# agakshat/spacefortress

Measured on NVIDIA B200. Metric: env-steps/sec with 84x84 obs, higher is better.
Workload: dtype f64

## Files before the change

spacefortress_b200/csrc/sf_kernels.cu:

```cuda
#include <cuda_runtime.h>
#include <stdio.h>
#include <stdlib.h>
#include <string.h>

#include <algorithm>
#include <mutex>
#include <string>
#include <vector>

#include "../../include/sf_b200.h"
#include "sf_geom.h"
#include "sf_render.cuh"
#include "sf_state.cuh"
#include "sf_step.cuh"
#include "sf_tables.h"

#define SF_BLOCK (32 * SF_RENDER_WARPS)

__host__ __device__ inline unsigned sf_hash3(unsigned seed, unsigned long long env, unsigned long long t) {
  unsigned long long z = (env * 0x9E3779B97F4A7C15ull) ^ (t * 0xC2B2AE3D27D4EB4Full) ^ ((unsigned long long)seed << 32 | 0x5Fu);
  z ^= z >> 30; z *= 0xBF58476D1CE4E5B9ull;
  z ^= z >> 27; z *= 0x94D049BB133111EBull;
  z ^= z >> 31;
  return (unsigned)(z >> 32);
}
__host__ __device__ inline int sf_hash_action(unsigned seed, unsigned long long env, unsigned long long t, int num_actions) {
  return (int)(((unsigned long long)sf_hash3(seed, env, t) * (unsigned)num_actions) >> 32);
}

__device__ __forceinline__ long long sf_warp_sum_ll(long long v) {
// ... 68 lines not shown
  unsigned long long* delta_stats;
  const unsigned char* draw_mask;
};
struct SfFeatArgs {
  float* out;
  int kind, cols;
};
enum SfRollMode { SF_ROLL_STEP, SF_ROLL_STEP_HOST_DELTA, SF_ROLL_DRAW };
template <int MODE>
__device__ __forceinline__ int sf_roll_ticks(const SfRollArgs& A) { return MODE == SF_ROLL_DRAW ? 1 : A.T; }

__device__ __forceinline__ int sf_step_keys(const SfDev& D, const SfRollArgs& A, int env, int t) {
  int a = A.actions ? A.actions[(size_t)t * D.n + env]
                    : sf_hash_action(A.action_seed, (unsigned long long)(D.first_global_env + env), (unsigned long long)(A.t0 + t), D.num_actions);
  return (A.flags & SF_FLAG_ACTIONS_ARE_KEYMASKS) ? (a & 15) : D.keymask_of_action[min(max(a, 0), D.num_actions - 1)];
}
__device__ __forceinline__ void sf_store_step_out(const SfDev& D, const SfRollArgs& A, int env, int t, const SfStepOut& o) {
  size_t oi = (size_t)t * D.n + env;
  if (A.reward) A.reward[oi] = o.reward;
  if (A.done) A.done[oi] = o.done;
  if (A.fortkill) A.fortkill[oi] = o.fort_kill;
  if (A.events) A.events[oi] = o.events;
}
__device__ __forceinline__ void sf_tick_env(const SfDev& D, const SfHot* H, const SfRollArgs& A, int env, int t, bool autoreset, SfEnv& e, SfStepOut& o) {
  const int km = sf_step_keys(D, A, env, t);
  sf_env_step(D, H, env, e, km, autoreset, (A.flags & SF_FLAG_RAW_REWARD) != 0, o);
  sf_store_step_out(D, A, env, t, o);
}

__device__ __noinline__ void sf_step_group(const SfDev& D, const SfRollArgs& A, int group, int t, SfEnvRec* recs) {
  const int lane = threadIdx.x & 31;
  const SfHot* H = &sf_block_smem().hot;
  const bool autoreset = !(A.flags & SF_FLAG_NO_AUTORESET);
  const int env = A.env0 + group * A.EB + lane;
  const bool mine = lane < A.EB && env < A.env0 + A.envn;
  SfEnv e;
  bool finished = false;
  unsigned shell_vis = 0;
  SF_ST_BEGIN(__ballot_sync(0xffffffffu, mine));
  SfStepSmem& SS = sf_block_smem().step;
  const bool first_tick = t == 0, last_tick = t == A.T - 1;
  if (mine) {
    if (first_tick) sf_load_env(D, env, e);
    else {
      e.pos = SS.pos[lane]; e.vel = SS.vel[lane];
      e.q0 = SS.q0[lane]; e.q1 = SS.q1[lane]; e.q2 = SS.q2[lane]; e.q3 = SS.q3[lane]; e.st3 = SS.st3[lane];
      e.d0 = SS.d0[lane]; e.d1 = SS.d1[lane]; e.d2 = SS.d2[lane];
    }
    SF_ST_USE(e.q0.x, e.q0.y);
    SF_ST(8);
    SfStepOut o;
    sf_tick_env(D, H, A, env, t, autoreset, e, o);
    finished = o.done && autoreset;
    shell_vis = o.shell_vis;
  }
  SF_ST_RESTART(0xffffffffu);
  if (__any_sync(0xffffffffu, finished)) {
    sf_accumulate_episode(D, env, e, finished, lane);
    if (finished) { sf_new_game(D, H, env, e); shell_vis = 0; }
  }
  if (mine) {
    if (last_tick) sf_store_env(D, env, e);
    else {
      SS.pos[lane] = e.pos; SS.vel[lane] = e.vel;
      SS.q0[lane] = e.q0; SS.q1[lane] = e.q1; SS.q2[lane] = e.q2; SS.q3[lane] = e.q3; SS.st3[lane] = e.st3;
      if ((t & 7) == 7) sf_flush_stats(D, env, e);
      SS.d0[lane] = e.d0; SS.d1[lane] = e.d1; SS.d2[lane] = e.d2;
    }
    sf_make_env_rec(e, env, shell_vis, recs[lane]);
  } else recs[lane].env = -1;
  __syncwarp();
  SF_ST(15);
}

__device__ __forceinline__ void sf_load_group(const SfDev& D, const SfRollArgs& A, int group, SfEnvRec* recs) {
  const int lane = threadIdx.x & 31;
  const int env = A.env0 + group * A.EB + lane;
  const bool mine = lane < A.EB && env < A.env0 + A.envn && (!A.draw_mask || A.draw_mask[env]);
  if (mine) {
    SfEnv e;
    sf_load_env(D, env, e);
    sf_make_env_rec(e, env, sf_visible_shells(D, env, (unsigned)e.q0.y), recs[lane]);
  } else recs[lane].env = -1;
  __syncwarp();
}

template <int MODE>
__device__ __forceinline__ void sf_stepper_role(const SfDev& D, const SfRollArgs& A) {
  const int lane = threadIdx.x & 31;
  SfBlockSmem& B = sf_block_smem();
  const bool native = (A.flags & SF_FLAG_NATIVE_OBS) != 0;
  int stage = 0, group = blockIdx.x;
#pragma unroll 1
  for (int k = 0; group < A.ngroups; k = (k + 1) % SF_NEXT_GROUPS) {
    if (lane == 0) B.next_group[k] = A.sched ? (int)gridDim.x + atomicAdd(&A.sched->next_group, 1) : group + (int)gridDim.x;
    sf_stepper_ticks(D, B, lane, native, sf_roll_ticks<MODE>(A), stage, [&](int t, SfStagePrep& Tm, int h) {
      if constexpr (MODE == SF_ROLL_DRAW) sf_load_group(D, A, group, Tm.env);
      else sf_step_group(D, A, group, t, &Tm.env[32 * h]);
    });
    group = B.next_group[k];
  }
  sf_stepper_drain(stage);
  if (lane == 0 && A.sched) {
    __threadfence();
    if (atomicAdd(&A.sched->done, 1) == (int)gridDim.x - 1) { A.sched->next_group = 0; A.sched->done = 0; __threadfence(); }
  }
}
template <int MODE>
__device__ __noinline__ void sf_rollout_stepper(const SfDev& D, const SfRollArgs& A) { sf_stepper_role<MODE>(D, A); }

template <int MODE>
__device__ __forceinline__ void sf_rollout_drawer(const SfDev& D, const SfRollArgs& A) {
  const int lane = threadIdx.x & 31;
  SfBlockSmem& B = sf_block_smem();
  SfWarpSmem& W = sf_my_smem();
  SfFrameOut out;
  out.native = (A.flags & SF_FLAG_NATIVE_OBS) ? 1 : 0;
  out.obs_bytes = out.native ? (size_t)SF_NAT_H * SF_NAT_W : (size_t)84 * 84;
  out.obs = A.obs;
  out.tick_bytes = MODE == SF_ROLL_DRAW ? 0 : (size_t)D.n * out.obs_bytes;
  SfStageState st;
// ... 352 lines not shown
  D.st1[i] = make_int4(r.stats[4], r.stats[5], r.stats[6], r.stats[7]);
  D.st2[i] = make_int4(r.stats[8], r.stats[9], r.stats[10], r.stats[11]);
  e.st3.x = r.stats[12];
  for (int s = 0; s < SF_MAX_MISSILES; s++) if ((r.missile_mask >> s) & 1) {
    D.mpos[(size_t)s * D.n_pad + i] = make_double2(r.missile_x[s], r.missile_y[s]);
    D.mang[(size_t)s * D.n_pad + i] = (short)(int)r.missile_angle[s];
  }
  for (int s = 0; s < SF_DEV_SHELLS; s++) if ((r.shell_mask >> s) & 1) {
    D.spos[(size_t)s * D.n_pad + i] = make_double2(r.shell_x[s], r.shell_y[s]);
    D.svel[(size_t)s * D.n_pad + i] = make_double2(r.shell_vx[s], r.shell_vy[s]);
    D.sang[(size_t)s * D.n_pad + i] = r.shell_angle[s];
  }
  sf_forget_render_caches(D, i);
  sf_store_env(D, i, e);
}

#define SF_BLOB_CHUNKS (SF_ENV_BLOB_BYTES / 16)
#define SF_BLOB_PITCH (SF_BLOB_CHUNKS + 1)
#define SF_BLOB_BLOCKS_PER_SM 8
enum { SF_BO_POS = 16, SF_BO_VEL = 32, SF_BO_Q = 48, SF_BO_ST = 112, SF_BO_MPOS = 176, SF_BO_SPOS = 496, SF_BO_SVEL = 560,
       SF_BO_SANG = 624, SF_BO_MANG = 656, SF_BO_RNG = 696, SF_BO_END = 820 };
static_assert(SF_BO_MANG + 2 * SF_MAX_MISSILES == SF_BO_RNG && SF_BO_RNG + 4 * SF_RNG_WORDS == SF_BO_END, "blob layout");
static_assert(SF_BO_END <= SF_ENV_BLOB_BYTES && SF_ENV_BLOB_BYTES % 16 == 0, "blob size");

__device__ __forceinline__ void sf_cp_async(void* smem, const void* gmem, int bytes) {
  const unsigned s = (unsigned)__cvta_generic_to_shared(smem);
  if (bytes == 16) asm volatile("cp.async.cg.shared.global [%0], [%1], 16;\n" ::"r"(s), "l"(gmem) : "memory");
  else if (bytes == 8) asm volatile("cp.async.ca.shared.global [%0], [%1], 8;\n" ::"r"(s), "l"(gmem) : "memory");
  else asm volatile("cp.async.ca.shared.global [%0], [%1], 4;\n" ::"r"(s), "l"(gmem) : "memory");
}
__device__ __forceinline__ void sf_cp_async_wait() { asm volatile("cp.async.wait_all;\n" ::: "memory"); }

__global__ void __launch_bounds__(32) sf_save_envs_kernel(SfDev D, int gametype, const int* __restrict__ idx, int count, int4* __restrict__ blob) {
  __shared__ int4 tile[32 * SF_BLOB_PITCH];
  const int lane = threadIdx.x;
  const size_t np = (size_t)D.n_pad;
  int4* row = tile + lane * SF_BLOB_PITCH;
  char* rb = reinterpret_cast<char*>(row);
  const int4 z = make_int4(0, 0, 0, 0);
  for (int base = blockIdx.x * 32; base < count; base += gridDim.x * 32) {
    const int k = base + lane;
    const int i = k < count ? (idx ? idx[k] : k) : -1;
    if (i >= 0 && i < D.n) {
      const int4 q0 = D.q0[i];
      const unsigned pm = (unsigned)q0.y;
      row[0] = make_int4((int)SF_ENV_BLOB_MAGIC, SF_ENV_BLOB_VERSION, gametype, 0);
      sf_cp_async(rb + SF_BO_POS, &D.pos[i], 16);
      sf_cp_async(rb + SF_BO_VEL, &D.vel[i], 16);
      row[SF_BO_Q / 16] = q0;
      sf_cp_async(rb + SF_BO_Q + 16, &D.q1[i], 16);
      sf_cp_async(rb + SF_BO_Q + 32, &D.q2[i], 16);
      sf_cp_async(rb + SF_BO_Q + 48, &D.q3[i], 16);
      sf_cp_async(rb + SF_BO_ST, &D.st0[i], 16);
      sf_cp_async(rb + SF_BO_ST + 16, &D.st1[i], 16);
// ... 235 lines not shown
  d.autoturn = (gt == 1 || gt == 3);
  bool test = gt >= 2;
  d.shaped = !test;
  d.destroy_fortress = test ? 100 : 1;
  d.death_penalty = test ? 100 : 1;
  d.missile_penalty = test ? 2.0f : (float)0.05;
  d.num_actions = na;
  for (int i = 0; i < 16; i++) d.keymask_of_action[i] = i < na ? km[i] : 0;
  d.first_global_env = 0;

  h->h_tab = new SfTables();
  char err[256] = {0};
  if (sf_build_tables(h->h_tab, err, sizeof(err))) { std::string m = err; delete h->h_tab; delete h; return fail(SF_ERR_INVALID, "table build failed: " + m); }

  auto bail = [&](const char* what, cudaError_t ce) { std::string m = std::string(what) + ": " + cudaGetErrorString(ce); sf_destroy(h); return fail(SF_ERR_CUDA, m); };
  cudaError_t ce;
  h->slab_bytes = layout(d, nullptr);
  if ((ce = cudaMalloc(&h->slab, h->slab_bytes)) != cudaSuccess) return bail("cudaMalloc state slab", ce);
  layout(d, (char*)h->slab);
  if ((ce = cudaMalloc(&h->d_sched, sizeof(SfSched))) != cudaSuccess) return bail("cudaMalloc scheduler state", ce);
  if ((ce = cudaMemset(h->d_sched, 0, sizeof(SfSched))) != cudaSuccess) return bail("cudaMemset scheduler state", ce);
  if ((ce = cudaMemset(h->slab, 0, h->slab_bytes)) != cudaSuccess) return bail("cudaMemset state slab", ce);
  if ((ce = cudaMemcpy((void*)d.tab, h->h_tab, sizeof(SfTables), cudaMemcpyHostToDevice)) != cudaSuccess) return bail("upload tables", ce);
  if ((ce = cudaFuncSetAttribute(sf_rollout_kernel<SF_ROLL_STEP>, cudaFuncAttributeMaxDynamicSharedMemorySize, (int)SF_RENDER_SMEM_BYTES(SF_RENDER_WARPS))) != cudaSuccess) return bail("shared memory opt-in (rollout)", ce);
  if ((ce = cudaFuncSetAttribute(sf_rollout_kernel<SF_ROLL_STEP_HOST_DELTA>, cudaFuncAttributeMaxDynamicSharedMemorySize, (int)SF_RENDER_SMEM_BYTES(SF_RENDER_WARPS))) != cudaSuccess) return bail("shared memory opt-in (rollout, host delta)", ce);
  if ((ce = cudaFuncSetAttribute(sf_rollout_kernel<SF_ROLL_DRAW>, cudaFuncAttributeMaxDynamicSharedMemorySize, (int)SF_RENDER_SMEM_BYTES(SF_RENDER_WARPS))) != cudaSuccess) return bail("shared memory opt-in (rollout, draw)", ce);
  if ((ce = cudaFuncSetAttribute(sf_pack_static_kernel, cudaFuncAttributeMaxDynamicSharedMemorySize, (int)SF_RENDER_SMEM_BYTES(SF_RENDER_WARPS))) != cudaSuccess) return bail("shared memory opt-in (pack)", ce);
  if ((ce = cudaFuncSetAttribute(sf_save_envs_kernel, cudaFuncAttributePreferredSharedMemoryCarveout, (int)cudaSharedmemCarveoutMaxShared)) != cudaSuccess) return bail("shared memory carveout (save envs)", ce);
  if ((ce = cudaFuncSetAttribute(sf_load_envs_kernel, cudaFuncAttributePreferredSharedMemoryCarveout, (int)cudaSharedmemCarveoutMaxShared)) != cudaSuccess) return bail("shared memory carveout (load envs)", ce);
  sf_pack_static_kernel<<<1, SF_BLOCK, SF_RENDER_SMEM_BYTES(SF_RENDER_WARPS)>>>(d, const_cast<unsigned char*>(d.static_image));
  if ((ce = cudaGetLastError()) != cudaSuccess) return bail("static image kernel launch", ce);
  sf_seed_kernel<<<(d.n + 127) / 128, 128>>>(d, nullptr);
  if ((ce = cudaGetLastError()) != cudaSuccess) return bail("seed kernel launch", ce);
  if ((ce = cudaDeviceSynchronize()) != cudaSuccess) return bail("seed kernel", ce);
  *out = h;
  return SF_OK;
}

extern "C" int sf_destroy(sf_handle* h) {
  if (!h) return SF_OK;
  cudaSetDevice(h->device);
  if (h->slab) cudaFree(h->slab);
  if (h->d_actions) cudaFree(h->d_actions);
  if (h->d_obs) cudaFree(h->d_obs);
  if (h->d_reward) cudaFree(h->d_reward);
  if (h->d_done) cudaFree(h->d_done);
  if (h->d_kill) cudaFree(h->d_kill);
// ... 62 lines not shown
      if (render) {
        const size_t o = (size_t)t * n;
        s.actions = a.actions ? a.actions + o : nullptr; s.t0 = a.t0 + t;
        s.reward = a.reward ? a.reward + o : nullptr; s.done = a.done ? a.done + o : nullptr;
        s.fortkill = a.fortkill ? a.fortkill + o : nullptr; s.events = a.events ? a.events + o : nullptr;
      }
      if (f.out) sf_step_repeat_kernel<true><<<blocks, SF_STEP_ONLY_BLOCK, 0, st>>>(d, s, f, h->action_repeat);
      else sf_step_repeat_kernel<false><<<blocks, SF_STEP_ONLY_BLOCK, 0, st>>>(d, s, f, h->action_repeat);
      CUDA_TRY(cudaGetLastError());
      if (render) {
        SfRollArgs r = {};
        r.T = 1; r.obs = a.obs + (size_t)t * n * per; r.flags = a.flags; r.env0 = a.env0; r.envn = a.envn;
        if (int rc = launch_rollout(h, r, st, true)) return rc;
      }
    }
    return SF_OK;
  }
  if (render) {
    int blocks;
    group_shape(h, a.envn, &a.EB, &a.ngroups, &blocks);
    a.sched = (!draw && a.env0 == 0 && a.envn == d.n && !a.host_obs) ? h->d_sched : nullptr;
    if (draw) sf_rollout_kernel<SF_ROLL_DRAW><<<blocks, SF_BLOCK, SF_RENDER_SMEM_BYTES(SF_RENDER_WARPS), st>>>(d, a);
    else if (a.host_obs) sf_rollout_kernel<SF_ROLL_STEP_HOST_DELTA><<<blocks, SF_BLOCK, SF_RENDER_SMEM_BYTES(SF_RENDER_WARPS), st>>>(d, a);
    else sf_rollout_kernel<SF_ROLL_STEP><<<blocks, SF_BLOCK, SF_RENDER_SMEM_BYTES(SF_RENDER_WARPS), st>>>(d, a);
  } else {
    const int blocks = (a.envn + SF_STEP_ONLY_BLOCK - 1) / SF_STEP_ONLY_BLOCK;
    if (f.out) sf_step_only_kernel<true><<<blocks, SF_STEP_ONLY_BLOCK, 0, st>>>(d, a, f);
    else sf_step_only_kernel<false><<<blocks, SF_STEP_ONLY_BLOCK, 0, st>>>(d, a, f);
  }
  CUDA_TRY(cudaGetLastError());
  return SF_OK;
}

#include <cuda_bf16.h>
#define SF_PI_THREADS 192
template <bool F32>
__global__ void __launch_bounds__(SF_PI_THREADS) sf_policy_input_kernel(const unsigned char* __restrict__ frames, long long fstride, int n, const int* __restrict__ valid,
                                                                       uint4* __restrict__ out) {
  __shared__ unsigned tile[2][4 * 4 * 21];
  __shared__ unsigned lut[256];
  const int env = blockIdx.x, tid = threadIdx.x;
  for (int v = tid; v < 256; v += SF_PI_THREADS) {
    if (F32) lut[v] = __float_as_uint(__fmul_rn((float)v, __fdiv_rn(1.0f, 255.0f)));
    else { const __nv_bfloat16 h = __float2bfloat16_rn(__fdiv_rn((float)v, 255.0f)); lut[v] = *reinterpret_cast<const unsigned short*>(&h); }
  }
  const int nvalid = min(max(valid[env], 0), 4);
  const unsigned char* base = frames + (long long)env * (84 * 84);
// ... 415 lines not shown
```

spacefortress_b200/csrc/sf_render.cuh:

```cuda
#pragma once
#include "sf_geom.h"
#include "sf_probe.cuh"
#include "sf_state.cuh"
#include "sf_tables.h"

#define SF_BATCH_QUADS 32
#define SF_MAX_GROUPS 256
#define SF_PATCH_STRIDE 32
#define SF_PATCH_BYTES (36 * 32)
#define SF_WIN_MAX_W 31
#define SF_WIN_MAX_H 34
#define SF_YBIAS 4096
#define SF_TAG_SHIP 0
#define SF_TAG_PROJECTILE 1
#define SF_SPAN_NONE 0xFFFFFFFFu
#define SF_QF_IRREGULAR 2

#define SF_RENDER_WARPS 24
#define SF_FORT_LIST_SMEM 48
#define SF_GROUP_ENVS 32
#define SF_STAGE_TICKS 2
#define SF_STAGE_SLOTS (SF_GROUP_ENVS * SF_STAGE_TICKS)
#define SF_ROUND_STROKES (8 * (SF_RENDER_WARPS - 1))
#define SF_CELLS_SHIP 144
// ... 100 lines not shown
  asm volatile("bar.arrive %0, %1;" :: "r"(3 + sg), "r"(32 * SF_RENDER_WARPS) : "memory");
}
__device__ __forceinline__ void sf_stage_full_wait(int sg) {
  SF_BT_BEGIN();
  asm volatile("bar.sync %0, %1;" :: "r"(3 + sg), "r"(32 * SF_RENDER_WARPS) : "memory");
  SF_BT(0);
}
__device__ __forceinline__ void sf_stage_empty_arrive(int sg) {
  asm volatile("bar.arrive %0, %1;" :: "r"(3 + SF_PREP_SLOTS + sg), "r"(32 * SF_RENDER_WARPS) : "memory");
}
__device__ __forceinline__ void sf_stage_empty_wait(int sg) {
  SF_BT_BEGIN();
  asm volatile("bar.sync %0, %1;" :: "r"(3 + SF_PREP_SLOTS + sg), "r"(32 * SF_RENDER_WARPS) : "memory");
  SF_BT(2);
}
__device__ __forceinline__ void sf_render_sync() {
  SF_BT_BEGIN();
  asm volatile("bar.sync 2, %0;" :: "r"(32 * (SF_RENDER_WARPS - 1)) : "memory");
  SF_BT(1);
}
__device__ __forceinline__ SfWarpSmem& sf_warp_smem(int warp) { return reinterpret_cast<SfWarpSmem*>(sf_smem_raw + sizeof(SfBlockSmem))[warp]; }
__device__ __forceinline__ SfWarpSmem& sf_my_smem() { return sf_warp_smem(threadIdx.x >> 5); }
#define SF_RENDER_SMEM_BYTES(warps) (sizeof(SfBlockSmem) + sizeof(SfWarpSmem) * (warps))

__device__ __forceinline__ int sf_warp_min(int v) {
#pragma unroll
  for (int o = 16; o; o >>= 1) v = min(v, __shfl_xor_sync(0xffffffffu, v, o));
  return v;
}
__device__ __forceinline__ int sf_warp_max(int v) {
#pragma unroll
  for (int o = 16; o; o >>= 1) v = max(v, __shfl_xor_sync(0xffffffffu, v, o));
  return v;
}
__device__ __forceinline__ int sf_div_small(int a, int b, float inv_b) {
  return __float2int_rz(((float)a + 0.5f) * inv_b);
}
__device__ __forceinline__ int sf_div15(int d) { return (d * 2185) >> 15; }

__device__ __forceinline__ void sf_block_smem_fill(const SfTables* T) {
  SfBlockSmem& B = sf_block_smem();
  for (int k = threadIdx.x; k < 168; k += blockDim.x) {
    const SfTap t = k < 84 ? T->xtap[k] : T->ytap[k - 84];
    int4 v = make_int4(t.si | (t.cnt << 8), __float_as_int(t.a[0]), __float_as_int(t.a[1]), __float_as_int(t.a[2]));
    if (k < 84) B.xtap[k] = v; else B.ytap[k - 84] = v;
  }
// ... 698 lines not shown
      for (int u = 0; u < 8; u++) {
        const int k = lane + 32 * u, w = k & 7;
        if (((rows >> (k >> 3)) & 1u) && w >= wfull0 && w < wfull1) *reinterpret_cast<unsigned*>(dst + (k >> 3) * 84 + 4 * w) = v[u];
      }
      if ((rows >> lane) & 1u) {
        const int wl = wfull0 - 1, wr = wfull1;
        if (wl >= 0) {
          const unsigned x = __ldcg(&src[lane * 8 + wl]);
          unsigned char* p = dst + lane * 84 + 4 * wl;
#pragma unroll
          for (int b = 0; b < 4; b++) { const int c = ja + 4 * wl + b; if (c >= j0 && c <= j1) p[b] = (unsigned char)(x >> (8 * b)); }
        }
        if (wr != wl && ja + 4 * wr <= j1) {
          const unsigned x = __ldcg(&src[lane * 8 + wr]);
          unsigned char* p = dst + lane * 84 + 4 * wr;
#pragma unroll
          for (int b = 0; b < 4; b++) { const int c = ja + 4 * wr + b; if (c >= j0 && c <= j1) p[b] = (unsigned char)(x >> (8 * b)); }
        }
      }
    }
  }
}

__device__ __forceinline__ void sf_gather_strokes(const SfDev& D, SfStagePrep& Tm, int lane, int h) {
  const int slot = 32 * h + lane;
  const SfEnvRec& rec = Tm.env[slot];
  if (slot >= Tm.r0 && slot < Tm.r1 && rec.env >= 0) {
    const int env = rec.env, np = D.n_pad;
    const unsigned core = rec.core;
    SfStrokeRec* S = &Tm.stroke[rec.s0];
    if (core & SF_CORE_SHIP_ALIVE) { S->x = rec.px; S->y = rec.py; S->desc = 0 | ((int)(core & SF_CORE_ANGLE_MASK) << 2) | (slot << 12); S++; }
    for (unsigned m = rec.pmask & SF_PMASK_MISSILES; m;) {
      const int k0 = __ffs(m) - 1; m &= m - 1;
      const int k1 = m ? __ffs(m) - 1 : k0; m &= m - 1;
      const int k2 = m ? __ffs(m) - 1 : k0; m &= m - 1;
      const double2 p0 = D.mpos[(size_t)k0 * np + env], p1 = D.mpos[(size_t)k1 * np + env], p2 = D.mpos[(size_t)k2 * np + env];
      const int a0 = D.mang[(size_t)k0 * np + env], a1 = D.mang[(size_t)k1 * np + env], a2 = D.mang[(size_t)k2 * np + env];
      S->x = p0.x; S->y = p0.y; S->desc = 1 | (a0 << 2) | (slot << 12); S++;
      if (k1 != k0) { S->x = p1.x; S->y = p1.y; S->desc = 1 | (a1 << 2) | (slot << 12); S++; }
      if (k2 != k0) { S->x = p2.x; S->y = p2.y; S->desc = 1 | (a2 << 2) | (slot << 12); S++; }
    }
    for (unsigned m = (unsigned)rec.shell_vis; m; m &= m - 1) {
      const int k = __ffs(m) - 1;
      const double2 p = D.spos[(size_t)k * np + env];
      int angle = __double2int_rz(D.sang[(size_t)k * np + env]);
      if (angle >= 360) angle -= 360;
      S->x = p.x; S->y = p.y; S->desc = 2 | (angle << 2) | (slot << 12); S++;
    }
  }
  __syncwarp();
}

__device__ __forceinline__ void sf_phase_strokes(const SfDev& D, SfBlockSmem& B, SfWarpSmem& W, int lane, int wi, int nw, int nst, int sg) {
  const SfTables* T = D.tab;
  const SfStagePrep& Tm = sf_prep(sg);
  const int chunk = Tm.chunk;
  const int be = Tm.build_env;
  if (be >= 0) sf_phase_exp_items(D, be, lane, nw - 1 - wi, nw, sg);
  const int s = wi * chunk;
  if (s < nst) {
    const int slot = lane >> 2;
    const bool valid = slot < chunk && s + slot < nst;
    const int idx = s + slot;
    int kind = -1, angle = 0;
    double x = 0, y = 0;
    if (valid) {
      const SfStrokeRec& S = Tm.stroke[idx];
      x = S.x; y = S.y; kind = S.desc & 3; angle = (S.desc >> 2) & 1023;
// ... 99 lines not shown
    for (int k = 0; k < SF_PREP_SLOTS * SF_STAGE_TICKS; k++) {
      const int j = k / SF_STAGE_TICKS, hh = k - j * SF_STAGE_TICKS;
      if (j == cur && hh >= h) continue;
      const SfEnvRec& o = ring[j].env[32 * hh + lane];
      if (o.env != r.env || (o.core & SF_CORE_SHIP_ALIVE)) continue;
      if (o.life == r.life) building = 0;
      if (o.life != r.life || sf_expo_key(o) != key) refresh = false;
    }
    if (!native) {
      const bool same = mx == r.life && (my & 0x0FFFFFFFu) == key;
      if (same) { if (!building) building |= (int)(my >> 28) << 4; }
      else atomicExch(reinterpret_cast<unsigned long long*>(&D.expo_meta[r.env]), (unsigned long long)r.life | ((unsigned long long)key << 32));
    }
    r.building = building | (refresh ? 2 : 0);
  }
  __syncwarp();
}

struct SfStageState {
  int stage;
  int prev_used;
};

template <class Prep>
__device__ __forceinline__ void sf_prepare_first_round(const SfDev& D, SfBlockSmem& B, int sg, int lane, int t, int nt, SfFrameOut out, Prep prep) {
  SfStagePrep& Tm = B.prep[sg];
  const bool native = out.native != 0;
  SF_BT_BEGIN();
  prep(t, Tm, 0);
  SF_BT(3);
  sf_publish_recs(D, B.prep, sg, lane, 0, native);
  SF_BT(4);
  SfScanState S;
  sf_scan_begin(S);
  sf_scan_half(Tm, lane, 0, 0, S);
  sf_scan_finish(Tm, lane, 0, S);
  SF_BT(5);
  sf_gather_strokes(D, Tm, lane, 0);
  SF_BT(6);
  int nticks = 1;
  if (nt > 1 && !Tm.more) {
    prep(t + 1, Tm, 1);
    SF_BT(3);
    sf_publish_recs(D, B.prep, sg, lane, 1, native);
    SF_BT(4);
    sf_scan_half(Tm, lane, 1, 0, S);
    sf_scan_finish(Tm, lane, 0, S);
    SF_BT(5);
    sf_gather_strokes(D, Tm, lane, 1);
    SF_BT(6);
    nticks = 2;
  }
  if (lane == 0) Tm.nticks = nticks;
  __syncwarp();
  SF_BT(7);
}

__device__ __forceinline__ int sf_draw_stage(const SfDev& D, SfBlockSmem& B, SfWarpSmem& W, int lane, const SfFrameOut& out, int sg) {
  const int warp = threadIdx.x >> 5;
  const int wi = warp - 1, nw = SF_RENDER_WARPS - 1;
  const SfStagePrep& Tm = B.prep[sg];
  SfStagePool& P = B.pool;
  const int r0 = Tm.r0, r1 = Tm.r1, nst = Tm.nstrokes;
  const bool base_issuer = !out.native && wi == nw - 1;
  if (base_issuer) {
#pragma unroll 1
    for (int e = r0 + lane; e < r1; e += 32) sf_env_base_issue(B, e, out, sg);
  }
  sf_phase_strokes(D, B, W, lane, wi, nw, nst, sg);
  if (!out.native) {
    if (base_issuer) {
      asm volatile("cp.async.bulk.wait_group 0;" ::: "memory");
// ... 26 lines not shown
      sf_phase_window(D, B, W, lane, t, netask, out, sg);
    }
  } else {
#pragma unroll 1
    for (int t = wi; t < (r1 - r0) * 12; t += nw) sf_phase_native_tile(D, B, W, lane, r0 + t / 12, t % 12, out, sg);
  }
  return used;
}


__device__ __forceinline__ int sf_stepper_claim(int stage) {
  const int sg = stage % SF_PREP_SLOTS;
  SF_TL(4);
  if (stage >= SF_PREP_SLOTS) sf_stage_empty_wait(sg);
  SF_TL(5);
  return sg;
}
__device__ __forceinline__ void sf_stepper_drain(int stage) {
#pragma unroll 1
  for (int s = max(stage - SF_PREP_SLOTS, 0); s < stage; s++)
    asm volatile("bar.sync %0, %1;" :: "r"(3 + SF_PREP_SLOTS + s % SF_PREP_SLOTS), "r"(32 * SF_RENDER_WARPS) : "memory");
}

template <class Prep>
__device__ __forceinline__ void sf_stepper_ticks(const SfDev& D, SfBlockSmem& B, int lane, bool native, int T, int& stage, Prep prep) {
  SfFrameOut out;
  out.obs = nullptr; out.obs_bytes = 0; out.tick_bytes = 0; out.native = native ? 1 : 0;
  int sg = sf_stepper_claim(stage);
  sf_prepare_first_round(D, B, sg, lane, 0, T, out, prep);
  SF_TL(3);
  int t = 0;
#pragma unroll 1
  for (;;) {
    sf_stage_full_arrive(sg);
    stage++;
    const SfStagePrep& Tm = B.prep[sg];
    const bool more = Tm.more != 0;
    const int nticks = Tm.nticks;
    if (!more && t + nticks >= T) break;
    const int nx = sf_stepper_claim(stage);
    SfStagePrep& Nx = B.prep[nx];
    if (more) {
#pragma unroll
      for (int h = 0; h < SF_STAGE_TICKS; h++) Nx.env[32 * h + lane] = Tm.env[32 * h + lane];
      if (lane == 0) Nx.nticks = nticks;
      __syncwarp();
      sf_round_scan(Nx, lane, Tm.r1, SF_GROUP_ENVS * nticks);
      sf_gather_strokes(D, Nx, lane, nticks - 1);
    } else {
      sf_prepare_first_round(D, B, nx, lane, t + nticks, T - (t + nticks), out, prep);
      t += nticks;
    }
    sg = nx;
  }
  SF_TL(7);
}

__device__ __forceinline__ void sf_drawer_ticks(const SfDev& D, SfBlockSmem& B, SfWarpSmem& W, int lane, SfFrameOut out, int T, SfStageState& st) {
  unsigned char* const obs0 = out.obs;
  int t = 0;
#pragma unroll 1
  for (;;) {
    const int sg = st.stage;
    SF_TL(4);
    sf_stage_full_wait(sg);
    SF_TL(5);
    const SfStagePrep& Tm = B.prep[sg];
    const bool more = Tm.more != 0;
    const int nticks = Tm.nticks;
    const bool last = !more && t + nticks >= T;
    {
      const int nz = (st.prev_used + 1) >> 1;
      for (int k = threadIdx.x - 32; k < nz; k += 32 * (SF_RENDER_WARPS - 1)) reinterpret_cast<unsigned*>(B.pool.cells)[k] = 0u;
// ... 12 lines not shown
```

spacefortress_b200/csrc/sf_state.cuh:

```cuda
#pragma once
#include <cuda_runtime.h>
#include <stdint.h>

#include "sf_tables.h"

#define SF_DEV_SHELLS 4
#define SF_RNG_WORDS 31

#define SF_CORE_ANGLE_MASK 0x1FFu
#define SF_CORE_FANG_SHIFT 9
#define SF_CORE_FLAST_SHIFT 15
#define SF_CORE_SHIP_ALIVE (1u << 21)
#define SF_CORE_FORT_ALIVE (1u << 22)
#define SF_CORE_FIRE (1u << 23)
#define SF_CORE_THRUST (1u << 24)
#define SF_CORE_LEFT (1u << 25)
#define SF_CORE_RIGHT (1u << 26)
#define SF_PMASK_MISSILES 0xFFFFFu
#define SF_PMASK_SHELL_SHIFT 20

struct SfDev {
  int n;
  int n_pad;
  double2* pos;
// ... 5 lines not shown
  int4* st0;
  int4* st1;
  int4* st2;
  int4* st3;
  double2* mpos;
  short* mang;
  double2* spos;
  double2* svel;
  double* sang;
  unsigned* rng;
  unsigned char* expc;
  unsigned* expstamp;
  unsigned char* expo;
  uint2* expo_meta;
  unsigned long long* epi;
  const SfTables* tab;
  const unsigned char* static_image;
  int autoturn, shaped, destroy_fortress, death_penalty;
  float missile_penalty;
  int num_actions;
  int keymask_of_action[16];
  long long first_global_env;
};
```

spacefortress_b200/csrc/sf_step.cuh:

```cuda
#pragma once
#include "sf_geom.h"
#include "sf_state.cuh"
#include "../../include/sf_b200.h"
#include "sf_probe.cuh"

#define SF_TICK_MS 34
#define SF_GAME_TIME 180000
#define SF_GAME_TICKS 5295

struct SfStepOut {
  int reward;
  unsigned events;
  bool done, fort_kill;
  unsigned shell_vis;
};

struct SfEnv {
  double2 pos, vel;
  int4 q0, q1, q2, q3, st3;
  unsigned d0, d1, d2;
};
#define SF_ST_INC(word, comp) ((word) += 1u << (8 * (comp)))

__device__ __forceinline__ void sf_load_env(const SfDev& D, int i, SfEnv& e) {
// ... 147 lines not shown
  e.st3.y = sp.w; e.st3.z += calls;
  e.pos = make_double2((double)sp.x, (double)sp.y);
  e.vel = make_double2(H->ship_start_vx, H->ship_start_vy);
  e.q0.x = (e.q0.x & ~SF_CORE_ANGLE_MASK) | (unsigned)sp.z | SF_CORE_SHIP_ALIVE;
}

__device__ inline void sf_new_game(const SfDev& D, const SfHot* H, int i, SfEnv& e) {
  e.q0 = make_int4(0, 0, 0, 0);
  sf_spawn_ship(D, H, i, e);
  e.q0.x |= SF_CORE_FORT_ALIVE | (18u << SF_CORE_FANG_SHIFT);
  e.q1 = make_int4(0, 250, 0, e.q1.w);
  e.q2 = make_int4(0, 0, 0, 0);
  e.q3 = make_int4(0, 0, 0, 0);
  D.st0[i] = make_int4(0, 0, 0, 0); D.st1[i] = make_int4(0, 0, 0, 0); D.st2[i] = make_int4(0, 0, 0, 0);
  e.d0 = 0u; e.d1 = 0u; e.d2 = 0u;
  e.st3.x = 0;
}

__device__ __forceinline__ int sf_first_free(unsigned mask, int n) {
  unsigned freebits = ~mask & ((1u << n) - 1u);
  return freebits ? __ffs(freebits) - 1 : -1;
}

__device__ inline void sf_env_step(const SfDev& D, const SfHot* T, int i, SfEnv& e, int keymask, bool autoreset, bool raw_reward, SfStepOut& out) {
  const int np = D.n_pad;
  SF_ST_BEGIN(__activemask());
  float rew = 0.f;
  unsigned ev = 0;
  unsigned core = (unsigned)e.q0.x;
  if (D.autoturn) keymask &= (SF_KEY_FIRE | SF_KEY_THRUST);

  {
    bool pressed = keymask & SF_KEY_FIRE, flag = core & SF_CORE_FIRE;
    if (pressed && !flag) {
      if (core & SF_CORE_SHIP_ALIVE) {
        int slot = sf_first_free((unsigned)e.q0.y & SF_PMASK_MISSILES, SF_MAX_MISSILES);
        if (slot >= 0) {
          e.q0.y |= 1 << slot;
          D.mpos[(size_t)slot * np + i] = e.pos;
          D.mang[(size_t)slot * np + i] = (short)(core & SF_CORE_ANGLE_MASK);
          ev |= SF_EV_MISSILE_FIRED;
          sf_reward(e, rew, -D.missile_penalty);
        }
      }
      core |= SF_CORE_FIRE; e.q2.x = 0; SF_ST_INC(e.d1, 3); ev |= SF_EV_PRESS_FIRE;
    } else if (!pressed && flag) { core &= ~SF_CORE_FIRE; e.q2.x = 0; }
    pressed = keymask & SF_KEY_THRUST; flag = core & SF_CORE_THRUST;
    if (pressed && !flag) { core |= SF_CORE_THRUST; e.q2.y = 0; SF_ST_INC(e.d2, 0); ev |= SF_EV_PRESS_THRUST; }
    else if (!pressed && flag) { core &= ~SF_CORE_THRUST; e.q2.y = 0; }
    if (!D.autoturn) {
      pressed = keymask & SF_KEY_LEFT; flag = core & SF_CORE_LEFT;
      if (pressed && !flag) { core |= SF_CORE_LEFT; e.q2.z = 0; SF_ST_INC(e.d2, 1); ev |= SF_EV_PRESS_LEFT; }
      else if (!pressed && flag) { core &= ~SF_CORE_LEFT; e.q2.z = 0; }
      pressed = keymask & SF_KEY_RIGHT; flag = core & SF_CORE_RIGHT;
      if (pressed && !flag) { core |= SF_CORE_RIGHT; e.q2.w = 0; SF_ST_INC(e.d2, 2); ev |= SF_EV_PRESS_RIGHT; }
      else if (!pressed && flag) { core &= ~SF_CORE_RIGHT; e.q2.w = 0; }
    }
  }
  e.q0.x = (int)core;

  if (!(core & SF_CORE_SHIP_ALIVE) && e.q0.z >= 1000) {
    sf_spawn_ship(D, T, i, e);
    e.q0.w = 0;
// ... 31 lines not shown
  }

  SF_ST(10);
  {
    if (!(core & SF_CORE_FORT_ALIVE) && e.q1.x > 1000) {
      e.q0.w = 0; core |= SF_CORE_FORT_ALIVE; ev |= SF_EV_FORTRESS_RESPAWN;
    }
    if (core & SF_CORE_SHIP_ALIVE) {
      const double fdy = SF_DSUB(e.pos.y, SF_FORT_Y), fdx = SF_DSUB(e.pos.x, SF_FORT_X);
      int sect = sf_ceil_angle<10>(T, fdy, fdx, false) / 10;
      if (sect >= 36) sect -= 36;
      unsigned last = (core >> SF_CORE_FLAST_SHIFT) & 63u;
      core = (core & ~(63u << SF_CORE_FANG_SHIFT)) | ((unsigned)sect << SF_CORE_FANG_SHIFT);
      if ((unsigned)sect != last) {
        core = (core & ~(63u << SF_CORE_FLAST_SHIFT)) | ((unsigned)sect << SF_CORE_FLAST_SHIFT);
        e.q0.w = 0;
      }
      if (e.q0.w >= 1000 && (core & SF_CORE_FORT_ALIVE)) {
        int slot = sf_first_free(((unsigned)e.q0.y >> SF_PMASK_SHELL_SHIFT) & 0xFu, SF_DEV_SHELLS);
        if (slot >= 0) {
          double a = sf_rad2deg(sf_atan2(T, fdy, fdx));
          if (a < 0) a = SF_DADD(a, 360.0);
          e.q0.y |= 1 << (SF_PMASK_SHELL_SHIFT + slot);
          D.spos[(size_t)slot * np + i] = make_double2(SF_FORT_X, SF_FORT_Y);
          D.svel[(size_t)slot * np + i] = sf_shell_velocity(a);
          D.sang[(size_t)slot * np + i] = a;
          ev |= SF_EV_FORTRESS_FIRED;
        }
        e.q0.w = 0;
      }
    }
    e.q0.x = (int)core;
  }

  SF_ST(11);
  const double thr_ship = T->touch2[0], thr_fort = T->touch2[1], thr_hide = T->touch2[2];
  unsigned vis = 0;
  for (unsigned m = ((unsigned)e.q0.y >> SF_PMASK_SHELL_SHIFT) & 0xFu; m; m &= m - 1) {
    int s = __ffs(m) - 1;
    double2 p = D.spos[(size_t)s * np + i], v = D.svel[(size_t)s * np + i];
    p.x = SF_DADD(p.x, v.x); p.y = SF_DADD(p.y, v.y);
    D.spos[(size_t)s * np + i] = p;
    if ((e.q0.x & SF_CORE_SHIP_ALIVE) && sf_dist2(p.x, p.y, e.pos.x, e.pos.y) <= thr_ship) {
      e.q0.y &= ~(1 << (SF_PMASK_SHELL_SHIFT + s));
      sf_kill_ship(e); sf_reward(e, rew, -(float)D.death_penalty); SF_ST_INC(e.d0, 2);
      ev |= SF_EV_SHELL_HIT_SHIP | SF_EV_COL_SHELL_SHIP;
    } else if (sf_outside(p.x, p.y)) {
      e.q0.y &= ~(1 << (SF_PMASK_SHELL_SHIFT + s));
    } else if (sf_dist2(p.x, p.y, SF_FORT_X, SF_FORT_Y) > thr_hide) vis |= 1u << s;
  }
  out.shell_vis = vis;

  SF_ST(12);
  for (unsigned m = (unsigned)e.q0.y & SF_PMASK_MISSILES; m; m &= m - 1) {
    int s = __ffs(m) - 1;
    double2 p = D.mpos[(size_t)s * np + i];
    int ang = D.mang[(size_t)s * np + i];
    p.x = SF_DADD(p.x, SF_DMUL(20.0, T->cs[ang][0]));
    p.y = SF_DADD(p.y, SF_DMUL(20.0, T->cs[ang][1]));
    D.mpos[(size_t)s * np + i] = p;
    if (sf_dist2(p.x, p.y, SF_FORT_X, SF_FORT_Y) <= thr_fort) {
      e.q0.y &= ~(1 << s);
      ev |= SF_EV_COL_MISSILE_FORTRESS;
      if (e.q0.x & SF_CORE_FORT_ALIVE) {
        ev |= SF_EV_HIT_FORTRESS;
        if (e.q1.y >= 250) {
          e.q1.z += 1; ev |= SF_EV_VLNER_INCREASED; SF_ST_INC(e.d2, 3);
          if (e.q1.z > e.st3.x) e.st3.x = e.q1.z;
        } else {
          if (e.q1.z >= 11) {
            e.q0.x &= ~SF_CORE_FORT_ALIVE; e.q1.x = 0;
            sf_reward(e, rew, (float)D.destroy_fortress);
            ev |= SF_EV_FORTRESS_DESTROYED; SF_ST_INC(e.d1, 1);
          } else { ev |= SF_EV_VLNER_RESET; SF_ST_INC(e.d1, 0); }
          e.q1.z = 0;
        }
        e.q1.y = 0;
      } else ev |= SF_EV_HIT_DEAD_FORTRESS;
    } else if (sf_outside(p.x, p.y)) {
      e.q0.y &= ~(1 << s);
      sf_reward(e, rew, -0.0f);
      SF_ST_INC(e.d1, 2); ev |= SF_EV_MISSED_SHOT;
    }
// ... 28 lines not shown
```

Baseline: 160.3 million.

## Keep projectile state in shared memory across rollout ticks

```diff
diff --git a/spacefortress_b200/csrc/sf_kernels.cu b/spacefortress_b200/csrc/sf_kernels.cu
--- a/spacefortress_b200/csrc/sf_kernels.cu
+++ b/spacefortress_b200/csrc/sf_kernels.cu
@@ -6,6 +6,7 @@
 #include <algorithm>
 #include <mutex>
 #include <string>
+#include <type_traits>
 #include <vector>
 
 #include "../../include/sf_b200.h"
@@ -120,12 +121,61 @@
   if (A.fortkill) A.fortkill[oi] = o.fort_kill;
   if (A.events) A.events[oi] = o.events;
 }
+template <class Proj = SfProjGlobal>
 __device__ __forceinline__ void sf_tick_env(const SfDev& D, const SfHot* H, const SfRollArgs& A, int env, int t, bool autoreset, SfEnv& e, SfStepOut& o) {
   const int km = sf_step_keys(D, A, env, t);
-  sf_env_step(D, H, env, e, km, autoreset, (A.flags & SF_FLAG_RAW_REWARD) != 0, o);
+  sf_env_step<Proj>(D, H, env, e, km, autoreset, (A.flags & SF_FLAG_RAW_REWARD) != 0, o);
   sf_store_step_out(D, A, env, t, o);
 }
 
+__device__ __forceinline__ void sf_cp_async(void* smem, const void* gmem, int bytes) {
+  const unsigned s = (unsigned)__cvta_generic_to_shared(smem);
+  if (bytes == 16) asm volatile("cp.async.cg.shared.global [%0], [%1], 16;\n" ::"r"(s), "l"(gmem) : "memory");
+  else if (bytes == 8) asm volatile("cp.async.ca.shared.global [%0], [%1], 8;\n" ::"r"(s), "l"(gmem) : "memory");
+  else asm volatile("cp.async.ca.shared.global [%0], [%1], 4;\n" ::"r"(s), "l"(gmem) : "memory");
+}
+__device__ __forceinline__ void sf_cp_async_wait() { asm volatile("cp.async.wait_all;\n" ::: "memory"); }
+
+__device__ __noinline__ void sf_proj_load(const SfDev& D, int env, unsigned pmask) {
+  SfProjSmem& P = sf_proj_smem();
+  const int lane = threadIdx.x & 31;
+  const size_t np = D.n_pad;
+  for (unsigned m = pmask & SF_PMASK_MISSILES; m; m &= m - 1) {
+    const int s = __ffs(m) - 1;
+    sf_cp_async(&P.mpos[s][lane], &D.mpos[s * np + env], 16);
+    sf_cp_async(&P.mang[s][lane], &D.mang[(s * np + env) & ~(size_t)1], 4);
+  }
+  for (unsigned m = (pmask >> SF_PMASK_SHELL_SHIFT) & 0xFu; m; m &= m - 1) {
+    const int s = __ffs(m) - 1;
+    sf_cp_async(&P.spos[s][lane], &D.spos[s * np + env], 16);
+    sf_cp_async(&P.svel[s][lane], &D.svel[s * np + env], 16);
+    sf_cp_async(&P.sang[s][lane], &D.sang[s * np + env], 8);
+  }
+  sf_cp_async_wait();
+  const int sh = (env & 1) ? 0 : 16;
+  for (unsigned m = pmask & SF_PMASK_MISSILES; m; m &= m - 1) {
+    const int s = __ffs(m) - 1;
+    P.mang[s][lane] = (int)((unsigned)P.mang[s][lane] << sh) >> 16;
+  }
+}
+__device__ __noinline__ void sf_proj_store(const SfDev& D, int env, unsigned pmask) {
+  const SfProjSmem& P = sf_proj_smem();
+  const int lane = threadIdx.x & 31;
+  const size_t np = D.n_pad;
+  for (unsigned m = pmask & SF_PMASK_MISSILES; m; m &= m - 1) {
+    const int s = __ffs(m) - 1;
+    D.mpos[s * np + env] = P.mpos[s][lane];
+    D.mang[s * np + env] = (short)P.mang[s][lane];
+  }
+  for (unsigned m = (pmask >> SF_PMASK_SHELL_SHIFT) & 0xFu; m; m &= m - 1) {
+    const int s = __ffs(m) - 1;
+    D.spos[s * np + env] = P.spos[s][lane];
+    D.svel[s * np + env] = P.svel[s][lane];
+    D.sang[s * np + env] = P.sang[s][lane];
+  }
+}
+
+template <class Proj>
 __device__ __noinline__ void sf_step_group(const SfDev& D, const SfRollArgs& A, int group, int t, SfEnvRec* recs) {
   const int lane = threadIdx.x & 31;
   const SfHot* H = &sf_block_smem().hot;
@@ -139,8 +189,10 @@
   SfStepSmem& SS = sf_block_smem().step;
   const bool first_tick = t == 0, last_tick = t == A.T - 1;
   if (mine) {
-    if (first_tick) sf_load_env(D, env, e);
-    else {
+    if (first_tick) {
+      sf_load_env(D, env, e);
+      if constexpr (std::is_same_v<Proj, SfProjShared>) sf_proj_load(D, env, (unsigned)e.q0.y);
+    } else {
       e.pos = SS.pos[lane]; e.vel = SS.vel[lane];
       e.q0 = SS.q0[lane]; e.q1 = SS.q1[lane]; e.q2 = SS.q2[lane]; e.q3 = SS.q3[lane]; e.st3 = SS.st3[lane];
       e.d0 = SS.d0[lane]; e.d1 = SS.d1[lane]; e.d2 = SS.d2[lane];
@@ -148,7 +200,7 @@
     SF_ST_USE(e.q0.x, e.q0.y);
     SF_ST(8);
     SfStepOut o;
-    sf_tick_env(D, H, A, env, t, autoreset, e, o);
+    sf_tick_env<Proj>(D, H, A, env, t, autoreset, e, o);
     finished = o.done && autoreset;
     shell_vis = o.shell_vis;
   }
@@ -158,8 +210,10 @@
     if (finished) { sf_new_game(D, H, env, e); shell_vis = 0; }
   }
   if (mine) {
-    if (last_tick) sf_store_env(D, env, e);
-    else {
+    if (last_tick) {
+      sf_store_env(D, env, e);
+      if constexpr (std::is_same_v<Proj, SfProjShared>) sf_proj_store(D, env, (unsigned)e.q0.y);
+    } else {
       SS.pos[lane] = e.pos; SS.vel[lane] = e.vel;
       SS.q0[lane] = e.q0; SS.q1[lane] = e.q1; SS.q2[lane] = e.q2; SS.q3[lane] = e.q3; SS.st3[lane] = e.st3;
       if ((t & 7) == 7) sf_flush_stats(D, env, e);
@@ -192,9 +246,10 @@
 #pragma unroll 1
   for (int k = 0; group < A.ngroups; k = (k + 1) % SF_NEXT_GROUPS) {
     if (lane == 0) B.next_group[k] = A.sched ? (int)gridDim.x + atomicAdd(&A.sched->next_group, 1) : group + (int)gridDim.x;
-    sf_stepper_ticks(D, B, lane, native, sf_roll_ticks<MODE>(A), stage, [&](int t, SfStagePrep& Tm, int h) {
+    using Proj = std::conditional_t<MODE == SF_ROLL_STEP, SfProjShared, SfProjGlobal>;
+    sf_stepper_ticks<Proj>(D, B, lane, native, sf_roll_ticks<MODE>(A), stage, [&](int t, SfStagePrep& Tm, int h) {
       if constexpr (MODE == SF_ROLL_DRAW) sf_load_group(D, A, group, Tm.env);
-      else sf_step_group(D, A, group, t, &Tm.env[32 * h]);
+      else sf_step_group<Proj>(D, A, group, t, &Tm.env[32 * h]);
     });
     group = B.next_group[k];
   }
@@ -593,14 +648,6 @@
        SF_BO_SANG = 624, SF_BO_MANG = 656, SF_BO_RNG = 696, SF_BO_END = 820 };
 static_assert(SF_BO_MANG + 2 * SF_MAX_MISSILES == SF_BO_RNG && SF_BO_RNG + 4 * SF_RNG_WORDS == SF_BO_END, "blob layout");
 static_assert(SF_BO_END <= SF_ENV_BLOB_BYTES && SF_ENV_BLOB_BYTES % 16 == 0, "blob size");
-
-__device__ __forceinline__ void sf_cp_async(void* smem, const void* gmem, int bytes) {
-  const unsigned s = (unsigned)__cvta_generic_to_shared(smem);
-  if (bytes == 16) asm volatile("cp.async.cg.shared.global [%0], [%1], 16;\n" ::"r"(s), "l"(gmem) : "memory");
-  else if (bytes == 8) asm volatile("cp.async.ca.shared.global [%0], [%1], 8;\n" ::"r"(s), "l"(gmem) : "memory");
-  else asm volatile("cp.async.ca.shared.global [%0], [%1], 4;\n" ::"r"(s), "l"(gmem) : "memory");
-}
-__device__ __forceinline__ void sf_cp_async_wait() { asm volatile("cp.async.wait_all;\n" ::: "memory"); }
 
 __global__ void __launch_bounds__(32) sf_save_envs_kernel(SfDev D, int gametype, const int* __restrict__ idx, int count, int4* __restrict__ blob) {
   __shared__ int4 tile[32 * SF_BLOB_PITCH];
@@ -882,7 +929,7 @@
   if ((ce = cudaMemset(h->d_sched, 0, sizeof(SfSched))) != cudaSuccess) return bail("cudaMemset scheduler state", ce);
   if ((ce = cudaMemset(h->slab, 0, h->slab_bytes)) != cudaSuccess) return bail("cudaMemset state slab", ce);
   if ((ce = cudaMemcpy((void*)d.tab, h->h_tab, sizeof(SfTables), cudaMemcpyHostToDevice)) != cudaSuccess) return bail("upload tables", ce);
-  if ((ce = cudaFuncSetAttribute(sf_rollout_kernel<SF_ROLL_STEP>, cudaFuncAttributeMaxDynamicSharedMemorySize, (int)SF_RENDER_SMEM_BYTES(SF_RENDER_WARPS))) != cudaSuccess) return bail("shared memory opt-in (rollout)", ce);
+  if ((ce = cudaFuncSetAttribute(sf_rollout_kernel<SF_ROLL_STEP>, cudaFuncAttributeMaxDynamicSharedMemorySize, (int)SF_ROLL_STEP_SMEM_BYTES)) != cudaSuccess) return bail("shared memory opt-in (rollout)", ce);
   if ((ce = cudaFuncSetAttribute(sf_rollout_kernel<SF_ROLL_STEP_HOST_DELTA>, cudaFuncAttributeMaxDynamicSharedMemorySize, (int)SF_RENDER_SMEM_BYTES(SF_RENDER_WARPS))) != cudaSuccess) return bail("shared memory opt-in (rollout, host delta)", ce);
   if ((ce = cudaFuncSetAttribute(sf_rollout_kernel<SF_ROLL_DRAW>, cudaFuncAttributeMaxDynamicSharedMemorySize, (int)SF_RENDER_SMEM_BYTES(SF_RENDER_WARPS))) != cudaSuccess) return bail("shared memory opt-in (rollout, draw)", ce);
   if ((ce = cudaFuncSetAttribute(sf_pack_static_kernel, cudaFuncAttributeMaxDynamicSharedMemorySize, (int)SF_RENDER_SMEM_BYTES(SF_RENDER_WARPS))) != cudaSuccess) return bail("shared memory opt-in (pack)", ce);
@@ -991,7 +1038,7 @@
     a.sched = (!draw && a.env0 == 0 && a.envn == d.n && !a.host_obs) ? h->d_sched : nullptr;
     if (draw) sf_rollout_kernel<SF_ROLL_DRAW><<<blocks, SF_BLOCK, SF_RENDER_SMEM_BYTES(SF_RENDER_WARPS), st>>>(d, a);
     else if (a.host_obs) sf_rollout_kernel<SF_ROLL_STEP_HOST_DELTA><<<blocks, SF_BLOCK, SF_RENDER_SMEM_BYTES(SF_RENDER_WARPS), st>>>(d, a);
-    else sf_rollout_kernel<SF_ROLL_STEP><<<blocks, SF_BLOCK, SF_RENDER_SMEM_BYTES(SF_RENDER_WARPS), st>>>(d, a);
+    else sf_rollout_kernel<SF_ROLL_STEP><<<blocks, SF_BLOCK, SF_ROLL_STEP_SMEM_BYTES, st>>>(d, a);
   } else {
     const int blocks = (a.envn + SF_STEP_ONLY_BLOCK - 1) / SF_STEP_ONLY_BLOCK;
     if (f.out) sf_step_only_kernel<true><<<blocks, SF_STEP_ONLY_BLOCK, 0, st>>>(d, a, f);
diff --git a/spacefortress_b200/csrc/sf_render.cuh b/spacefortress_b200/csrc/sf_render.cuh
--- a/spacefortress_b200/csrc/sf_render.cuh
+++ b/spacefortress_b200/csrc/sf_render.cuh
@@ -146,6 +146,23 @@
 __device__ __forceinline__ SfWarpSmem& sf_warp_smem(int warp) { return reinterpret_cast<SfWarpSmem*>(sf_smem_raw + sizeof(SfBlockSmem))[warp]; }
 __device__ __forceinline__ SfWarpSmem& sf_my_smem() { return sf_warp_smem(threadIdx.x >> 5); }
 #define SF_RENDER_SMEM_BYTES(warps) (sizeof(SfBlockSmem) + sizeof(SfWarpSmem) * (warps))
+
+struct __align__(16) SfProjSmem {
+  double2 mpos[SF_MAX_MISSILES][SF_GROUP_ENVS];
+  int mang[SF_MAX_MISSILES][SF_GROUP_ENVS];
+  double2 spos[SF_DEV_SHELLS][SF_GROUP_ENVS], svel[SF_DEV_SHELLS][SF_GROUP_ENVS];
+  double sang[SF_DEV_SHELLS][SF_GROUP_ENVS];
+};
+#define SF_ROLL_STEP_SMEM_BYTES (SF_RENDER_SMEM_BYTES(SF_RENDER_WARPS) + sizeof(SfProjSmem))
+__device__ __forceinline__ SfProjSmem& sf_proj_smem() { return *reinterpret_cast<SfProjSmem*>(sf_smem_raw + SF_RENDER_SMEM_BYTES(SF_RENDER_WARPS)); }
+struct SfProjShared {
+  static __device__ __forceinline__ double2& mpos(const SfDev&, int, int s, int) { return sf_proj_smem().mpos[s][threadIdx.x & 31]; }
+  static __device__ __forceinline__ int mang(const SfDev&, int, int s, int) { return sf_proj_smem().mang[s][threadIdx.x & 31]; }
+  static __device__ __forceinline__ void set_mang(const SfDev&, int, int s, int, int a) { sf_proj_smem().mang[s][threadIdx.x & 31] = a; }
+  static __device__ __forceinline__ double2& spos(const SfDev&, int, int s, int) { return sf_proj_smem().spos[s][threadIdx.x & 31]; }
+  static __device__ __forceinline__ double2& svel(const SfDev&, int, int s, int) { return sf_proj_smem().svel[s][threadIdx.x & 31]; }
+  static __device__ __forceinline__ double& sang(const SfDev&, int, int s, int) { return sf_proj_smem().sang[s][threadIdx.x & 31]; }
+};
 
 __device__ __forceinline__ int sf_warp_min(int v) {
 #pragma unroll
@@ -890,6 +907,7 @@
   }
 }
 
+template <class Proj>
 __device__ __forceinline__ void sf_gather_strokes(const SfDev& D, SfStagePrep& Tm, int lane, int h) {
   const int slot = 32 * h + lane;
   const SfEnvRec& rec = Tm.env[slot];
@@ -902,16 +920,16 @@
       const int k0 = __ffs(m) - 1; m &= m - 1;
       const int k1 = m ? __ffs(m) - 1 : k0; m &= m - 1;
       const int k2 = m ? __ffs(m) - 1 : k0; m &= m - 1;
-      const double2 p0 = D.mpos[(size_t)k0 * np + env], p1 = D.mpos[(size_t)k1 * np + env], p2 = D.mpos[(size_t)k2 * np + env];
-      const int a0 = D.mang[(size_t)k0 * np + env], a1 = D.mang[(size_t)k1 * np + env], a2 = D.mang[(size_t)k2 * np + env];
+      const double2 p0 = Proj::mpos(D, np, k0, env), p1 = Proj::mpos(D, np, k1, env), p2 = Proj::mpos(D, np, k2, env);
+      const int a0 = Proj::mang(D, np, k0, env), a1 = Proj::mang(D, np, k1, env), a2 = Proj::mang(D, np, k2, env);
       S->x = p0.x; S->y = p0.y; S->desc = 1 | (a0 << 2) | (slot << 12); S++;
       if (k1 != k0) { S->x = p1.x; S->y = p1.y; S->desc = 1 | (a1 << 2) | (slot << 12); S++; }
       if (k2 != k0) { S->x = p2.x; S->y = p2.y; S->desc = 1 | (a2 << 2) | (slot << 12); S++; }
     }
     for (unsigned m = (unsigned)rec.shell_vis; m; m &= m - 1) {
       const int k = __ffs(m) - 1;
-      const double2 p = D.spos[(size_t)k * np + env];
-      int angle = __double2int_rz(D.sang[(size_t)k * np + env]);
+      const double2 p = Proj::spos(D, np, k, env);
+      int angle = __double2int_rz(Proj::sang(D, np, k, env));
       if (angle >= 360) angle -= 360;
       S->x = p.x; S->y = p.y; S->desc = 2 | (angle << 2) | (slot << 12); S++;
     }
@@ -1057,7 +1075,7 @@
   int prev_used;
 };
 
-template <class Prep>
+template <class Proj, class Prep>
 __device__ __forceinline__ void sf_prepare_first_round(const SfDev& D, SfBlockSmem& B, int sg, int lane, int t, int nt, SfFrameOut out, Prep prep) {
   SfStagePrep& Tm = B.prep[sg];
   const bool native = out.native != 0;
@@ -1071,7 +1089,7 @@
   sf_scan_half(Tm, lane, 0, 0, S);
   sf_scan_finish(Tm, lane, 0, S);
   SF_BT(5);
-  sf_gather_strokes(D, Tm, lane, 0);
+  sf_gather_strokes<Proj>(D, Tm, lane, 0);
   SF_BT(6);
   int nticks = 1;
   if (nt > 1 && !Tm.more) {
@@ -1082,7 +1100,7 @@
     sf_scan_half(Tm, lane, 1, 0, S);
     sf_scan_finish(Tm, lane, 0, S);
     SF_BT(5);
-    sf_gather_strokes(D, Tm, lane, 1);
+    sf_gather_strokes<Proj>(D, Tm, lane, 1);
     SF_BT(6);
     nticks = 2;
   }
@@ -1155,12 +1173,12 @@
     asm volatile("bar.sync %0, %1;" :: "r"(3 + SF_PREP_SLOTS + s % SF_PREP_SLOTS), "r"(32 * SF_RENDER_WARPS) : "memory");
 }
 
-template <class Prep>
+template <class Proj, class Prep>
 __device__ __forceinline__ void sf_stepper_ticks(const SfDev& D, SfBlockSmem& B, int lane, bool native, int T, int& stage, Prep prep) {
   SfFrameOut out;
   out.obs = nullptr; out.obs_bytes = 0; out.tick_bytes = 0; out.native = native ? 1 : 0;
   int sg = sf_stepper_claim(stage);
-  sf_prepare_first_round(D, B, sg, lane, 0, T, out, prep);
+  sf_prepare_first_round<Proj>(D, B, sg, lane, 0, T, out, prep);
   SF_TL(3);
   int t = 0;
 #pragma unroll 1
@@ -1179,9 +1197,9 @@
       if (lane == 0) Nx.nticks = nticks;
       __syncwarp();
       sf_round_scan(Nx, lane, Tm.r1, SF_GROUP_ENVS * nticks);
-      sf_gather_strokes(D, Nx, lane, nticks - 1);
+      sf_gather_strokes<Proj>(D, Nx, lane, nticks - 1);
     } else {
-      sf_prepare_first_round(D, B, nx, lane, t + nticks, T - (t + nticks), out, prep);
+      sf_prepare_first_round<Proj>(D, B, nx, lane, t + nticks, T - (t + nticks), out, prep);
       t += nticks;
     }
     sg = nx;
diff --git a/spacefortress_b200/csrc/sf_state.cuh b/spacefortress_b200/csrc/sf_state.cuh
--- a/spacefortress_b200/csrc/sf_state.cuh
+++ b/spacefortress_b200/csrc/sf_state.cuh
@@ -51,3 +51,12 @@
   int keymask_of_action[16];
   long long first_global_env;
 };
+
+struct SfProjGlobal {
+  static __device__ __forceinline__ double2& mpos(const SfDev& D, int np, int s, int i) { return D.mpos[(size_t)s * np + i]; }
+  static __device__ __forceinline__ int mang(const SfDev& D, int np, int s, int i) { return D.mang[(size_t)s * np + i]; }
+  static __device__ __forceinline__ void set_mang(const SfDev& D, int np, int s, int i, int a) { D.mang[(size_t)s * np + i] = (short)a; }
+  static __device__ __forceinline__ double2& spos(const SfDev& D, int np, int s, int i) { return D.spos[(size_t)s * np + i]; }
+  static __device__ __forceinline__ double2& svel(const SfDev& D, int np, int s, int i) { return D.svel[(size_t)s * np + i]; }
+  static __device__ __forceinline__ double& sang(const SfDev& D, int np, int s, int i) { return D.sang[(size_t)s * np + i]; }
+};
diff --git a/spacefortress_b200/csrc/sf_step.cuh b/spacefortress_b200/csrc/sf_step.cuh
--- a/spacefortress_b200/csrc/sf_step.cuh
+++ b/spacefortress_b200/csrc/sf_step.cuh
@@ -193,6 +193,7 @@
   return freebits ? __ffs(freebits) - 1 : -1;
 }
 
+template <class Proj = SfProjGlobal>
 __device__ inline void sf_env_step(const SfDev& D, const SfHot* T, int i, SfEnv& e, int keymask, bool autoreset, bool raw_reward, SfStepOut& out) {
   const int np = D.n_pad;
   SF_ST_BEGIN(__activemask());
@@ -208,8 +209,8 @@
         int slot = sf_first_free((unsigned)e.q0.y & SF_PMASK_MISSILES, SF_MAX_MISSILES);
         if (slot >= 0) {
           e.q0.y |= 1 << slot;
-          D.mpos[(size_t)slot * np + i] = e.pos;
-          D.mang[(size_t)slot * np + i] = (short)(core & SF_CORE_ANGLE_MASK);
+          Proj::mpos(D, np, slot, i) = e.pos;
+          Proj::set_mang(D, np, slot, i, (int)(core & SF_CORE_ANGLE_MASK));
           ev |= SF_EV_MISSILE_FIRED;
           sf_reward(e, rew, -D.missile_penalty);
         }
@@ -287,9 +288,9 @@
           double a = sf_rad2deg(sf_atan2(T, fdy, fdx));
           if (a < 0) a = SF_DADD(a, 360.0);
           e.q0.y |= 1 << (SF_PMASK_SHELL_SHIFT + slot);
-          D.spos[(size_t)slot * np + i] = make_double2(SF_FORT_X, SF_FORT_Y);
-          D.svel[(size_t)slot * np + i] = sf_shell_velocity(a);
-          D.sang[(size_t)slot * np + i] = a;
+          Proj::spos(D, np, slot, i) = make_double2(SF_FORT_X, SF_FORT_Y);
+          Proj::svel(D, np, slot, i) = sf_shell_velocity(a);
+          Proj::sang(D, np, slot, i) = a;
           ev |= SF_EV_FORTRESS_FIRED;
         }
         e.q0.w = 0;
@@ -303,9 +304,9 @@
   unsigned vis = 0;
   for (unsigned m = ((unsigned)e.q0.y >> SF_PMASK_SHELL_SHIFT) & 0xFu; m; m &= m - 1) {
     int s = __ffs(m) - 1;
-    double2 p = D.spos[(size_t)s * np + i], v = D.svel[(size_t)s * np + i];
+    double2 p = Proj::spos(D, np, s, i), v = Proj::svel(D, np, s, i);
     p.x = SF_DADD(p.x, v.x); p.y = SF_DADD(p.y, v.y);
-    D.spos[(size_t)s * np + i] = p;
+    Proj::spos(D, np, s, i) = p;
     if ((e.q0.x & SF_CORE_SHIP_ALIVE) && sf_dist2(p.x, p.y, e.pos.x, e.pos.y) <= thr_ship) {
       e.q0.y &= ~(1 << (SF_PMASK_SHELL_SHIFT + s));
       sf_kill_ship(e); sf_reward(e, rew, -(float)D.death_penalty); SF_ST_INC(e.d0, 2);
@@ -319,11 +320,11 @@
   SF_ST(12);
   for (unsigned m = (unsigned)e.q0.y & SF_PMASK_MISSILES; m; m &= m - 1) {
     int s = __ffs(m) - 1;
-    double2 p = D.mpos[(size_t)s * np + i];
-    int ang = D.mang[(size_t)s * np + i];
+    double2 p = Proj::mpos(D, np, s, i);
+    int ang = Proj::mang(D, np, s, i);
     p.x = SF_DADD(p.x, SF_DMUL(20.0, T->cs[ang][0]));
     p.y = SF_DADD(p.y, SF_DMUL(20.0, T->cs[ang][1]));
-    D.mpos[(size_t)s * np + i] = p;
+    Proj::mpos(D, np, s, i) = p;
     if (sf_dist2(p.x, p.y, SF_FORT_X, SF_FORT_Y) <= thr_fort) {
       e.q0.y &= ~(1 << s);
       ev |= SF_EV_COL_MISSILE_FORTRESS;
```

Measured after the change: 159.9 million, median of 6. About the same (-0.3%).
